# ytinyui/music2midi

Measured on AMD Instinct MI355X. Metric: decoded MIDI tokens/sec/node on 10 s clips, higher is better.
Workload: dtype bf16; 1 GPU; BASELINE configs[2]: full generate (log-mel + encoder + KV-cached greedy decode), bf16, batch 32 clips/GPU x 220500 samples, S=864, max_length 1024; global_batch=32, clips_per_gpu=32, rows_with_eos=0, parallelism=clip-sharded x1, weight_broadcast_bytes=0, world=1, backend=none

## Files before the change

music2midi_amd/csrc/decode.hip:

```cpp
#include "mma.h"
#include "t5.h"

#include <stdlib.h>
#include <type_traits>

namespace m2m {

#ifdef M2M_STAMPS
__device__ unsigned long long g_stamps[1 << 18];
__device__ unsigned int g_stamp_n;
#define M2M_STAMP(kid, phase)                                                                   \
  do {                                                                                          \
    if (threadIdx.x == 0 && blockIdx.x == 0 && blockIdx.y == 0) {                               \
      static_assert((phase) < 8, "phase");                                                      \
      if ((phase) == 0) m2m_stamp_base = atomicAdd(&g_stamp_n, 8u);                             \
      const unsigned long long tk = __builtin_amdgcn_s_memrealtime();                           \
      if (m2m_stamp_base + 8 <= (1u << 18))                                                     \
        g_stamps[m2m_stamp_base + (phase)] = ((unsigned long long)(kid) << 56) | ((unsigned long long)(phase) << 48) | (tk & 0xFFFFFFFFFFFFull); \
    }                                                                                           \
  } while (0)
#define M2M_STAMP_DECL unsigned int m2m_stamp_base = 0; (void)m2m_stamp_base;
#else
#define M2M_STAMP(kid, phase) do {} while (0)
#define M2M_STAMP_DECL
// ... 519 lines not shown
  int H, inner;
  DecState* state;
  const float* emb;
  unsigned long long* keys;
  int* finished;
  int64_t* tokens;
  const int* tok_row;
  int max_len, V, pad_id, eos_id;
  int book;
  const int* fin_skip;
  int fin_stride;
  const unsigned char* anc;
  int64_t anc_par;
  int anc_ld;
  int beam_nb;
};

typedef unsigned int m2m_u32x4 __attribute__((ext_vector_type(4)));
template <bool NT, typename V> __device__ inline V kv_load(const V* p) {
  if constexpr (NT) return __builtin_bit_cast(V, __builtin_nontemporal_load(reinterpret_cast<const m2m_u32x4*>(p)));
  else return *p;
}
#define M2M_KV_LOAD(p) kv_load<NT>(p)

template <typename T> __device__ inline float m2m_exp(float x) {
  if constexpr (sizeof(T) == 2) return __builtin_amdgcn_exp2f(x * 1.4426950408889634f);
  else return expf(x);
}

typedef __bf16 m2m_bf16x2 __attribute__((ext_vector_type(2)));
// ... 80 lines not shown
    if (lane == 0) red.lf[wave] = red.l[wave] * fw;
  }
  __syncthreads();
  if (tid < DK) {
    float s = 0.f, L = 0.f;
#pragma unroll
    for (int wv = 0; wv < 16; ++wv) {
      s += red.o[wv][tid];
      L += red.lf[wv];
    }
    put_in<T>(oh, tid, !(L <= 0.f) ? s / L : 0.f);
  }
  __syncthreads();
}

template <typename T, int C, int LPO, int WREG>
__device__ __forceinline__ void da_project(float (&acc)[C], const Vec16<T> (&w)[WREG], const T* wrow, int cnt, int part, const float* hn, int d) {
  constexpr int E = 16 / sizeof(T);
  using V16 = decltype(Vec16<T>().v);
#pragma unroll
  for (int c = 0; c < C; ++c) acc[c] = 0.f;
#pragma unroll
  for (int u = 0; u < WREG; ++u) {
    if (u < cnt) {
#pragma unroll
      for (int c = 0; c < C; ++c) acc[c] = chunk_dot<T>(w[u], hn + c * d, u * LPO + part, acc[c]);
    }
  }
  for (int i = WREG; i < cnt; i += 4) {
    Vec16<T> w2[4];
// ... 36 lines not shown
}

__device__ __forceinline__ void da_book_row(const DecAttnArgs& a, int b, int st_t, int st_done) {
  if (!st_done) {
    const int fin = a.finished[b];
    const int next = amax_key_token(a.keys[b], fin, a.V, a.pad_id);
    if (st_t < a.max_len) a.tokens[(int64_t)a.tok_row[b] * a.max_len + st_t] = next;
    const int nf = fin | (next == a.eos_id);
    a.finished[b] = nf;
    if (!nf) atomicAdd(&a.state->n_unfinished, 1);
    a.keys[b] = 0ull;
  }
  if (b == 0) a.state->t_copy = st_t;
}

template <typename T, bool SELF, bool NT, bool FETCH = false, bool BEAM = false>
__global__ __launch_bounds__(1024) void dec_attn_kernel(DecAttnArgs a) {
  static_assert(!FETCH || SELF, "only the layer-0 self-attention fetches its input row from the embedding table");
  static_assert(!(FETCH && BEAM), "the beam step is not headless");
  constexpr int E = 16 / sizeof(T);
  constexpr int LPR = DK / E;
  constexpr int KPW = 64 / LPR;
  constexpr int KPB = 16 * KPW;
  constexpr int NOUT = DK;
  constexpr int LPO = 16;
  constexpr int LPO2 = 8;
  constexpr int WMAX2 = 6;
#ifndef M2M_DA_PF_CROSS
#define M2M_DA_PF_CROSS 2
#endif
#ifndef M2M_DA_PF_SELF
#define M2M_DA_PF_SELF 2
#endif
#ifndef M2M_DA_REQUEST_FIRST
// ... 23 lines not shown
  const int hh = blockIdx.x, b = blockIdx.y;
  const int row_fin = a.fin_skip[(int64_t)b * a.fin_stride];
  const int sub = lane % LPR;
  const int kslot = wave * KPW + lane / LPR;
  const int bkv = (BEAM && !SELF) ? b / a.beam_nb : b;
  T* Kb = reinterpret_cast<T*>(a.Kc) + ((int64_t)bkv * a.H + hh) * a.kv_stride * DK;
  T* Vb = reinterpret_cast<T*>(a.Vc) + ((int64_t)bkv * a.H + hh) * a.kv_stride * DK;
  unsigned char* const ancl = reinterpret_cast<unsigned char*>(hn + a.d + (SELF ? a.bias_stride : 0));
  const int beam = (BEAM && SELF) ? b % a.beam_nb : 0;
  if constexpr (BEAM && SELF) {
    const unsigned char* ar = a.anc + (int64_t)(st_t & 1) * a.anc_par + (int64_t)b * a.anc_ld;
    const int na = min(max(st_t, 1), a.kv_stride);
    for (int j = tid; j < na; j += 1024) ancl[j] = j < st_t ? (unsigned char)min((int)ar[j], a.beam_nb - 1) : (unsigned char)beam;
    __syncthreads();
  }
  auto kvoff = [&](int key) -> int64_t {
    int64_t o = (int64_t)key * DK + sub * E;
    if constexpr (BEAM && SELF) o += ((int64_t)ancl[key] - beam) * ((int64_t)a.H * a.kv_stride * DK);
    return o;
  };

  const int xc = min(tid * 4, a.d - 4);
  const int on_ = min(tid >> 1, a.d - 1), opart = tid & 1;
  longlong2 xr0 = make_longlong2(0, 0), xr1 = make_longlong2(0, 0);
  xq_t xres = 0;
  unsigned long long kraw = 0;
  int fin0 = 0;
  if constexpr (FETCH) {
    kraw = a.keys[b];
    fin0 = a.finished[b];
  } else {
    xr0 = *reinterpret_cast<const longlong2*>(a.x + (int64_t)b * a.d + xc);
    xr1 = *reinterpret_cast<const longlong2*>(a.x + (int64_t)b * a.d + xc + 2);
    xres = a.x[(int64_t)b * a.d + on_];
  }
  const float4 gv = *reinterpret_cast<const float4*>(a.ln_w + xc);
  __builtin_amdgcn_sched_barrier(0);
  const int po = min(tid / LPO, NOUT - 1), part = tid % LPO;
  const int which = po / DK, dd = po - which * DK;
  const T* wrow = reinterpret_cast<const T*>(a.Wp) + ((int64_t)which * a.inner + hh * DK + dd) * a.d;
  const int cnt = a.d / E / LPO;
  Vec16<T> w[WMAX];
#pragma unroll
  for (int u = 0; u < WMAX; ++u) w[u].v = *reinterpret_cast<const V16*>(wrow + (min(u, cnt - 1) * LPO + part) * E);
  float* const biasl = hn + a.d;
  constexpr int BPT = 2;
  float bv[SELF ? BPT : 1];
  if (SELF) {
#pragma unroll
    for (int u = 0; u < BPT; ++u) bv[u] = a.bias[(int64_t)hh * a.bias_stride + min(tid + 1024 * u, a.bias_stride - 1)];
  }

  const int t = SELF ? (a.self_len_override > 0 ? a.self_len_override - 1 : st_t) : 0;
  const int n_prev = SELF ? t : a.n_keys;
  const int last = max(n_prev - 1, 0);

  Vec16<T> kv[PF], vv[PF];
#pragma unroll
  for (int u = 0; u < PF; ++u) {
    const int64_t off = kvoff(min(kslot + u * KPB, last));
    kv[u].v = M2M_KV_LOAD(reinterpret_cast<const V16*>(Kb + off));
    vv[u].v = M2M_KV_LOAD(reinterpret_cast<const V16*>(Vb + off));
  }
  __builtin_amdgcn_sched_barrier(0);
  const bool own_wave = wave * 256 < a.d;
  float4 xv = make_float4(0.f, 0.f, 0.f, 0.f);
  float eres = 0.f;
  float4 e4 = make_float4(0.f, 0.f, 0.f, 0.f);
  if constexpr (FETCH) {
    const int tok = amax_key_token(kraw, fin0, a.V, a.pad_id);
    const float* er = a.emb + (int64_t)tok * a.d;
    e4 = *reinterpret_cast<const float4*>(er + xc);
    eres = er[on_];
  }
  {
    const bool own = tid * 4 < a.d;
    if (own_wave) {
      if constexpr (FETCH) xv = e4;
      else xv = make_float4(xq_flt(xr0.x), xq_flt(xr0.y), xq_flt(xr1.x), xq_flt(xr1.y));
      float ss = own ? (xv.x * xv.x + xv.y * xv.y + xv.z * xv.z + xv.w * xv.w) : 0.f;
      ss = wave_sum(ss);
      if (lane == 0) redw[wave] = ss;
    } else if (lane == 0) {
      redw[wave] = 0.f;
    }
    __syncthreads();
    M2M_STAMP(6 + (SELF ? 1 : 0), 4);
    if (own) {
      float tot = 0.f;
#pragma unroll
      for (int wv = 0; wv < 16; ++wv) tot += redw[wv];
      const float rs = rsqrtf(tot / (float)a.d + a.eps);
      put_in<T>(hn, xc + 0, gv.x * (xv.x * rs));
      put_in<T>(hn, xc + 1, gv.y * (xv.y * rs));
      put_in<T>(hn, xc + 2, gv.z * (xv.z * rs));
      put_in<T>(hn, xc + 3, gv.w * (xv.w * rs));
    }
    __syncthreads();
    M2M_STAMP(6 + (SELF ? 1 : 0), 5);
  }

  {
    float q[1];
    da_project<T, 1, LPO>(q, w, wrow, cnt, part, hn, a.d);
#ifndef M2M_STAMPS_MERGE
    M2M_STAMP(6 + (SELF ? 1 : 0), 6);
#endif
    if (part == 0 && tid < NOUT * LPO) qs[dd] = q[0];
  }
  if (SELF) {
#pragma unroll
    for (int u = 0; u < BPT; ++u)
      if (tid + 1024 * u < a.bias_stride) biasl[tid + 1024 * u] = bv[u];
    for (int n = tid + 1024 * BPT; n < a.bias_stride; n += 1024) biasl[n] = a.bias[(int64_t)hh * a.bias_stride + n];
  }
  __syncthreads();
  M2M_STAMP(6 + (SELF ? 1 : 0), 1);

  constexpr int OCH = 32 / E;
  const T* woimg = reinterpret_cast<const T*>(a.Wo) + ((int64_t)hh * OCH * 2 * a.d + min(tid, 2 * a.d - 1)) * E;
  Vec16<T> wo[OCH];
#pragma unroll
  for (int u = 0; u < OCH; ++u) wo[u].v = *reinterpret_cast<const V16*>(woimg + (int64_t)u * 2 * a.d * E);
  const int o2 = tid >> 3, part2 = tid & 7;
  const int which2 = 1 + (o2 >> 6), dd2 = o2 & 63;
  const T* wrow2 = reinterpret_cast<const T*>(a.Wp) + ((int64_t)which2 * a.inner + hh * DK + dd2) * a.d;
  const int cnt2 = a.d / E / LPO2;
  Vec16<T> wkv[SELF ? WMAX2 : 1];
  if (SELF) {
#pragma unroll
    for (int u = 0; u < WMAX2; ++u) wkv[u].v = *reinterpret_cast<const V16*>(wrow2 + (min(u, cnt2 - 1) * LPO2 + part2) * E);
  }

  const int n_live = row_fin ? 0 : n_prev;
  float qv[E];
#pragma unroll
  for (int e = 0; e < E; ++e) qv[e] = qs[sub * E + e];
  DaSoftmax<T> sm;
  auto round = [&](const int k0, const int u, Vec16<T>& ks, Vec16<T>& vs, const int reissue ) {
    const int key = k0 + kslot + u * KPB;
    float s = 0.f;
#pragma unroll
    for (int e = 0; e < E; ++e) s = fmaf(qv[e], ks.get(e), s);
    s = group_sum<LPR>(s);
#if M2M_DA_REQUEST_FIRST
    float vrow[E];
#pragma unroll
    for (int e = 0; e < E; ++e) vrow[e] = vs.get(e);
    if (reissue == 1 || (reissue == 2 && k0 + (u + PF) * KPB < n_live)) {
      const int64_t off = kvoff(min(key + PF * KPB, last));
      ks.v = M2M_KV_LOAD(reinterpret_cast<const V16*>(Kb + off));
      vs.v = M2M_KV_LOAD(reinterpret_cast<const V16*>(Vb + off));
    }
    if (key < n_live) {
      if (SELF) s += biasl[t - key];
      sm.visit(s, vrow);
    }
#else
    if (key < n_live) {
      float vrow[E];
#pragma unroll
      for (int e = 0; e < E; ++e) vrow[e] = vs.get(e);
      if (SELF) s += biasl[t - key];
      sm.visit(s, vrow);
    }
    if (reissue == 1 || (reissue == 2 && k0 + (u + PF) * KPB < n_live)) {
      const int64_t off = kvoff(min(key + PF * KPB, last));
      ks.v = M2M_KV_LOAD(reinterpret_cast<const V16*>(Kb + off));
      vs.v = M2M_KV_LOAD(reinterpret_cast<const V16*>(Vb + off));
    }
#endif
  };
  int k0 = 0;
  for (; k0 + (2 * PF - 1) * KPB < n_live; k0 += PF * KPB) {
#pragma unroll
    for (int u = 0; u < PF; ++u) round(k0, u, kv[u], vv[u], 1);
  }
  for (; k0 < n_live; k0 += PF * KPB) {
#pragma unroll
    for (int u = 0; u < PF; ++u) round(k0, u, kv[u], vv[u], 2);
  }
  if (SELF) {
    float kvn[1];
    da_project<T, 1, LPO2>(kvn, wkv, wrow2, cnt2, part2, hn, a.d);
    if (part2 == 0) da_append_kv<T>(kvn[0], 0, which2, dd2, t, 0, Kb, Vb, kn, vn, !st_done);
    __syncthreads();
  }
  if (SELF && wave == 0 && lane < LPR) sm.visit_own(qv, kn, vn, biasl, sub);
  M2M_STAMP(6 + (SELF ? 1 : 0), 2);

  da_merge<T>(sm, red, oh, [&] {
#ifdef M2M_STAMPS_MERGE
    M2M_STAMP(6 + (SELF ? 1 : 0), 6);
#endif
  });
  M2M_STAMP(6 + (SELF ? 1 : 0), 7);
  da_out_row<T>(a, wo, oh, b, !st_done, true, [&] { return FETCH ? xq_fix_guarded(eres, a.state) : xres; });
  if (!SELF && a.book && hh == 0 && tid == 0) da_book_row(a, b, st_t, st_done);
  M2M_STAMP(6 + (SELF ? 1 : 0), 3);
}

#ifndef M2M_MC_PF_SELF
#define M2M_MC_PF_SELF 2
#endif
#ifndef M2M_MC_PF_CROSS
#define M2M_MC_PF_CROSS 2
#endif
#ifndef M2M_MC_ABL
#define M2M_MC_ABL 0
#endif
#ifndef M2M_MC_WAVES
#define M2M_MC_WAVES 4
#endif
template <typename T, bool SELF, bool NT, bool FETCH, int C, int CIF = 1, bool BEAM = false>
// ... 394 lines not shown
    else launch(s, no, fetch, beam);
  };
  if (a.beam_nb > 0) {
    if (self) by_nt(yes, no, yes);
    else by_nt(no, no, yes);
  } else if (self && a.emb) {
    by_nt(yes, yes, no);
  } else if (self) {
    by_nt(yes, no, no);
  } else {
    by_nt(no, no, no);
  }
}

template <typename T>
static void launch_dec_attn_t(bool self, bool nt, const DecAttnArgs& a, dim3 grid, size_t smem, hipStream_t st) {
  launch_dec_attn_form(self, nt, a, [&](auto s, auto n, auto f, auto bm) {
    hipLaunchKernelGGL((dec_attn_kernel<T, s.value, n.value, f.value, bm.value>), grid, dim3(1024), smem, st, a);
  });
}

template <typename T, int C>
static void launch_dec_attn_mc_t(bool self, bool nt, const DecAttnArgs& a, int nb, int cif, size_t smem, hipStream_t st) {
  const dim3 grid((unsigned)a.H, (unsigned)ceil_div(nb, C));
  launch_dec_attn_form(self, nt, a, [&](auto s, auto n, auto f, auto bm) {
    if constexpr (!s.value && !bm.value) {
      if (cif == 2) {
        hipLaunchKernelGGL((dec_attn_mc_kernel<T, false, n.value, false, C, 2>), grid, dim3(1024), smem, st, a, nb);
        return;
      }
    }
    hipLaunchKernelGGL((dec_attn_mc_kernel<T, s.value, n.value, f.value, C, 1, bm.value>), grid, dim3(1024), smem, st, a, nb);
  });
}

static int launch_dec_attn(int precision, bool self, bool nt, DecAttnArgs a, int B, int clips, int cif, hipStream_t st) {
  size_t smem = ((size_t)a.d * (size_t)clips + (self ? (size_t)a.bias_stride : 0)) * sizeof(float);
  if (self && a.beam_nb > 0) smem += (size_t)clips * a.kv_stride;
  M2M_REQUIRE(smem <= 24 * 1024, "decode attention: max_dec_len=%d too long for the LDS bias row%s (<= %d)", a.bias_stride,
              self && a.beam_nb > 0 ? " and ancestries" : "",
              (24 * 1024 - a.d * 4 * clips) / (self && a.beam_nb > 0 ? 4 + clips : 4));
  const bool bf = precision == M2M_PREC_BF16;
  if (clips == 1) {
    dim3 grid((unsigned)a.H, (unsigned)B);
    if (bf) launch_dec_attn_t<bf16_t>(self, nt, a, grid, smem, st);
    else launch_dec_attn_t<float>(self, nt, a, grid, smem, st);
  } else if (clips == 2) {
    if (bf) launch_dec_attn_mc_t<bf16_t, 2>(self, nt, a, B, cif, smem, st);
    else launch_dec_attn_mc_t<float, 2>(self, nt, a, B, cif, smem, st);
  } else if (clips == 4) {
    if (bf) launch_dec_attn_mc_t<bf16_t, 4>(self, nt, a, B, cif, smem, st);
    else launch_dec_attn_mc_t<float, 4>(self, nt, a, B, cif, smem, st);
  } else {
    set_error("decode attention: %d clips per workgroup not instantiated (1, 2, 4)", clips);
    return M2M_ERR_INVALID;
  }
  M2M_CHECK_HIP(hipGetLastError());
  return M2M_OK;
}

struct DecHeadArgs {
// ... 1023 lines not shown
    a.beam_nb = s->beam_nb;
    a.anc = s->anc + (int64_t)v.b0 * s->max_dec; a.anc_par = (int64_t)s->max_batch * s->max_dec; a.anc_ld = s->max_dec;
  }
  if (headless && layer == 0) {
    a.keys = s->keys + v.b0; a.finished = s->finished + v.b0; a.tokens = s->tokens; a.tok_row = s->tok_row + v.b0;
    a.max_len = s->max_dec; a.V = g.vocab_size; a.pad_id = g.pad_token_id; a.eos_id = g.eos_token_id;
    if (self) a.emb = m->shared; else a.book = 1;
  }
  if (self) {
    const size_t off = ((size_t)layer * kv_layer_elems(s, s->max_dec) + (size_t)v.b0 * H * s->max_dec * DK) * es;
    a.ln_w = L.ln0; a.Wp = L.wqkv; a.Wo = L.wo_img;
    a.Kc = (unsigned char*)s->self_k + off;
    a.Vc = (unsigned char*)s->self_v + off;
    a.kv_stride = s->max_dec; a.n_keys = 0; a.self_len_override = self_len;
    a.bias = s->dec_bias_tab; a.bias_stride = s->max_dec;
    return launch_dec_attn(m->precision, true, nt, a, v.nb, clips, s->sw.mc_cif, st);
  }
  const size_t per = (size_t)s->B * H * s->S * DK;
  const size_t voff = (size_t)(beam ? v.b0 / s->beam_nb : v.b0) * H * s->S * DK;
  a.ln_w = L.ln1; a.Wp = L.wcq; a.Wo = L.wco_img;
  a.Kc = (unsigned char*)s->cross_kv + (((size_t)layer * 2 + 0) * per + voff) * es;
  a.Vc = (unsigned char*)s->cross_kv + (((size_t)layer * 2 + 1) * per + voff) * es;
  a.kv_stride = s->S; a.n_keys = s->S; a.self_len_override = 0; a.bias = nullptr; a.bias_stride = 0;
  return launch_dec_attn(m->precision, false, nt, a, v.nb, clips, s->sw.mc_cif, st);
}

int decode_launch_step(m2m_session* s, const DecView& v, bool forced, float* logits_out, int Ld, hipStream_t st) {
  const m2m_model* m = s->m;
  const m2m_t5_geometry& g = m->g;
  const int P = m->precision;
  xq_t* xA = xbuf(s, v, 0);
  xq_t* xB = xbuf(s, v, 1);
  xq_t* xC = xbuf(s, v, 2);
  int rc;
  const bool headless = headless_for(s, forced);
  for (int l = 0; l < g.num_decoder_layers; ++l) {
    const DecLayerPacked& L = m->dec[l];
    if ((rc = decode_launch_attn(s, v, true, l, 0, st, headless, !forced))) return rc;
    if ((rc = decode_launch_attn(s, v, false, l, 0, st, headless, !forced))) return rc;
// ... 41 lines not shown
```

music2midi_amd/csrc/t5.h:

```cpp
#pragma once

#include "common.h"
#include "env.h"

#include <vector>

namespace m2m {

constexpr int DK = 64;

struct EncLayerPacked {
  const float* ln0;
  const void* wqkv;
  const void* wo;
  const float* ln1;
  const void* wi;
  const void* wo_ff;
};

struct DecLayerPacked {
  const float* ln0;
  const void* wqkv;
  const void* wo;
  const float* ln1;
  const void* wcq;
  const void* wco;
  const float* ln2;
  const void* wi;
  const void* wo_ff;
  const void* ff_img;
  const void* wo_img;
  const void* wco_img;
};

constexpr int FF_IMG_FRAG = 512;
constexpr int FF_IMG_WAVE = 12 * FF_IMG_FRAG;

}

struct m2m_model {
  m2m_t5_geometry g;
  int precision;
  int inner;
  int vocab_pad;
  size_t esize;
  void* blob = nullptr;
  int64_t blob_bytes = 0;
  std::vector<m2m::EncLayerPacked> enc;
  std::vector<m2m::DecLayerPacked> dec;
  const float* enc_final_ln = nullptr;
  const float* dec_final_ln = nullptr;
  const float* shared = nullptr;
  const void* lm_head = nullptr;
  const void* wckv = nullptr;
  std::vector<float> enc_rel_bias_host;
  std::vector<float> dec_rel_bias_host;
};

namespace m2m {

struct DecState {
  int t;
  int done;
  int out_len;
  int n_unfinished;
  int max_steps;
  int overflow;
  int t_copy;
  int zero;
// ... 117 lines not shown
inline const EncSwitches& enc_switches_now() { return tl_enc_switches ? *tl_enc_switches : process_enc_switches(); }

struct SessionSwitches {
  static int one_of_124(int c) { return (c == 1 || c == 2 || c == 4) ? c : 0; }
  static int zero_is_1(int c) { return c == 0 ? 1 : c; }
  EncSwitches enc = read_enc_switches();
  int attn_clips = env_int("M2M_DA_CLIPS", 0);
  int attn_clips_self = one_of_124(env_int("M2M_DA_CLIPS_SELF", 0));
  int ff_rows = env_int("M2M_DEC_FF_ROWS", 0);
  int ff_slices = env_int("M2M_DEC_FF_SLICES", 0);
  int mc_cif = zero_is_1(env_int("M2M_MC_CIF", 0));
  bool headless = env_on("M2M_HEADLESS");
  bool finished_skip = env_on("M2M_FINISHED_SKIP");
  int kv_resident_layers = env_int("M2M_KV_RESIDENT_LAYERS", -1);
  bool kv_resident_stagger = env_on("M2M_KV_RESIDENT_STAGGER");
};

constexpr int MAX_GROUPS = 8;

struct DecView {
  int b0, nb;
  DecState* state;
  int ord = 0, count = 1;
};

inline bool kv_layer_resident(int layer, int L, int resident, int ord, int count, bool stagger) {
  if (resident >= L) return true;
  if (resident <= 0) return false;
  const int first = (stagger && count == 2) ? (ord * resident) % L : 0;
  return (layer - first + L) % L < resident;
}

struct DecGroup {
  DecView view{0, 0, nullptr};
  DecState* state_host = nullptr;
  hipStream_t stream = nullptr;
  hipEvent_t ev_done = nullptr;
  hipGraphExec_t graph_exec = nullptr;
  struct GraphEntry { int key[10]; hipGraph_t graph; hipGraphExec_t exec; unsigned long long used; };
  std::vector<GraphEntry> graphs;
  unsigned long long graph_clock = 0;
};
}

struct m2m_session {
  const m2m_model* m;
  int max_batch, max_enc, max_dec;
  unsigned char* ws;
  int64_t ws_bytes;
  float* x_enc;
  void* h_enc;
  void* qkv_enc;
  void* vt_enc;
  void* attn_enc;
// ... 81 lines not shown
};
int launch_attn(int precision, const AttnArgs& a, bool causal, hipStream_t st);
int launch_transpose_v(int precision, const void* v, void* vt, int BH, int S, int Sp, hipStream_t st);
int launch_embed_rows(const int64_t* ids, const float* table, float* x, int M, int d, int V, int pad_id, hipStream_t st);
int launch_final_norm_f32(const float* x, const float* w, float* out_f32, void* out_T, int precision, int M, int d,
                          float eps, hipStream_t st);

int launch_convert(int precision, const float* src, void* dst, int64_t n, hipStream_t st);
int launch_interleave(int precision, const float* wi0, const float* wi1, void* dst, int dff, int d, int half,
                      hipStream_t st);
int launch_ff_image(int precision, const void* wi, const void* wo_ff, void* img, int dff, int d, hipStream_t st);
int launch_attn_out_image(int precision, const void* wo, void* img, int H, int d, hipStream_t st);
int launch_copy_f32(const float* src, float* dst, int64_t n, hipStream_t st);
int launch_fill_zero(void* dst, int64_t bytes, hipStream_t st);
int launch_checksum(const void* buf, int64_t bytes, unsigned long long* acc_dev, hipStream_t st);

int decode_init(m2m_session* s, const DecView& v, int max_steps, bool forced, hipStream_t st);
int decode_launch_step(m2m_session* s, const DecView& v, bool forced, float* logits_out, int Ld, hipStream_t st);
int decode_launch_attn(m2m_session* s, const DecView& v, bool self, int layer, int self_len, hipStream_t st, bool headless = false,
                       bool skip_finished = false);
int decode_move_rows(m2m_session* s, const int* src, const int* dst, int n, int t, hipStream_t st);
struct KvPolicy { bool nt; int resident; };
KvPolicy decode_kv_policy(const m2m_session* s);
bool decode_chains_may_drift(const m2m_session* s, int chains);
int decode_clear_self(m2m_session* s, const DecView& v, int t0, int t1, hipStream_t st);
int decode_finalize(m2m_session* s, const DecView& v, hipStream_t st);
constexpr int HEAD_GREEDY = 0, HEAD_SAMPLE = 1, HEAD_BEAM = 2;
constexpr int HEAD_PROCESSED = 4;
constexpr int HEAD_SCORED = 8;
constexpr int BEAM_MAX = 32;
// ... 9 lines not shown
```

music2midi_amd/csrc/t5_api.hip:

```cpp
#include "carver.h"
#include "env.h"
#include "t5.h"

#include <math.h>
#include <stdlib.h>
#include <string.h>
#include <algorithm>
#include <memory>
#include <vector>

using namespace m2m;

extern "C" int m2m_rel_bucket(int rel, int bidirectional, int num_buckets, int max_distance) {
  int bucket = 0;
  int nb = num_buckets;
  int n;
  if (bidirectional) {
    nb /= 2;
    if (rel > 0) bucket += nb;
    n = rel < 0 ? -rel : rel;
  } else {
    n = rel < 0 ? -rel : 0;
  }
  const int max_exact = nb / 2;
// ... 40 lines not shown
  auto T = [&](const void*& member, int64_t elems) { c.take(member, elems * es); };
  for (EncLayerPacked& L : m->enc) {
    F(L.ln0, d); T(L.wqkv, (int64_t)3 * inner * d); T(L.wo, (int64_t)d * inner);
    F(L.ln1, d); T(L.wi, (int64_t)2 * dff * d); T(L.wo_ff, (int64_t)d * dff);
  }
  for (DecLayerPacked& L : m->dec) {
    F(L.ln0, d); T(L.wqkv, (int64_t)3 * inner * d); T(L.wo, (int64_t)d * inner);
    F(L.ln1, d); T(L.wcq, (int64_t)inner * d); T(L.wco, (int64_t)d * inner);
    F(L.ln2, d); T(L.wi, (int64_t)2 * dff * d); T(L.wo_ff, (int64_t)d * dff); T(L.ff_img, (int64_t)3 * dff * d);
    T(L.wo_img, (int64_t)d * inner); T(L.wco_img, (int64_t)d * inner);
  }
  F(m->enc_final_ln, d); F(m->dec_final_ln, d);
  F(m->shared, (int64_t)V * d);
  T(m->lm_head, (int64_t)vocab_pad * d);
  T(m->wckv, (int64_t)Ld * 2 * inner * d);
  m->blob_bytes = c.off;
  hipError_t e = hipMalloc(&m->blob, (size_t)c.off);
  if (e != hipSuccess) {
    set_error("m2m_model_create: hipMalloc(%lld) failed: %s", (long long)c.off, hipGetErrorString(e));
    delete m;
    return M2M_ERR_NOMEM;
  }
  c.bind((unsigned char*)m->blob);
  int rc = M2M_OK;
  if (hipMemsetAsync(m->blob, 0, (size_t)c.off, st) != hipSuccess) { set_error("m2m_model_create: hipMemsetAsync failed"); rc = M2M_ERR_HIP; }
  auto at = [&](const void* member, int64_t part = 0) { return (unsigned char*)const_cast<void*>(member) + part * inner * d * (int64_t)es; };
  auto conv = [&](const float* src, void* dst, int64_t n) {
    if (rc == M2M_OK && !src) { set_error("m2m_model_create: null layer weight pointer"); rc = M2M_ERR_INVALID; }
    if (rc == M2M_OK) rc = launch_convert(precision, src, dst, n, st);
  };
// ... 21 lines not shown
    conv(s.q, at(L.wqkv, 0), (int64_t)inner * d); conv(s.k, at(L.wqkv, 1), (int64_t)inner * d); conv(s.v, at(L.wqkv, 2), (int64_t)inner * d);
    conv(s.o, at(L.wo), (int64_t)d * inner);
    conv(s.cq, at(L.wcq), (int64_t)inner * d);
    conv(s.co, at(L.wco), (int64_t)d * inner);
    if (rc == M2M_OK) rc = launch_attn_out_image(precision, L.wo, at(L.wo_img), g.num_heads, d, st);
    if (rc == M2M_OK) rc = launch_attn_out_image(precision, L.wco, at(L.wco_img), g.num_heads, d, st);
    interleave(s.wi0, s.wi1, L.wi, 8);
    conv(s.wo, at(L.wo_ff), (int64_t)d * dff);
    if (rc == M2M_OK) rc = launch_ff_image(precision, L.wi, L.wo_ff, at(L.ff_img), dff, d, st);
    conv(s.ck, at(m->wckv, l * 2 + 0), (int64_t)inner * d); conv(s.cv, at(m->wckv, l * 2 + 1), (int64_t)inner * d);
  }
  copyf(w->enc_final_ln, m->enc_final_ln, d); copyf(w->dec_final_ln, m->dec_final_ln, d);
  copyf(w->shared, m->shared, (int64_t)V * d);
  if (rc == M2M_OK) rc = launch_fill_zero(at(m->lm_head), (int64_t)vocab_pad * d * es, st);
  conv(w->lm_head, at(m->lm_head), (int64_t)V * d);
  m->enc_rel_bias_host.resize((size_t)g.num_buckets * g.num_heads);
  m->dec_rel_bias_host.resize((size_t)g.num_buckets * g.num_heads);
  hipError_t he = hipSuccess;
  if (rc == M2M_OK) he = hipMemcpyAsync(m->enc_rel_bias_host.data(), w->enc_rel_bias, m->enc_rel_bias_host.size() * 4, hipMemcpyDeviceToHost, st);
  if (rc == M2M_OK && he == hipSuccess) he = hipMemcpyAsync(m->dec_rel_bias_host.data(), w->dec_rel_bias, m->dec_rel_bias_host.size() * 4, hipMemcpyDeviceToHost, st);
  if (rc == M2M_OK && he == hipSuccess) he = hipStreamSynchronize(st);
  if (rc == M2M_OK && he != hipSuccess) { set_error("m2m_model_create: %s", hipGetErrorString(he)); rc = M2M_ERR_HIP; }
  if (rc != M2M_OK) {
    (void)hipFree(m->blob);
    delete m;
    return rc;
  }
  *out = m;
  return M2M_OK;
}
// ... 61 lines not shown
  c.take(s->hyp_tok, (int64_t)B * L * 8);
  c.take(s->score_dev, sizeof(ScoreParams));
  c.take(s->gram_dev, sizeof(GrammarParams));
  c.take(s->gram_state, (int64_t)B * sizeof(GrammarState));
}

int check_switches(const SessionSwitches& sw) {
  M2M_REQUIRE(sw.attn_clips == 0 || sw.attn_clips == 1 || sw.attn_clips == 2 || sw.attn_clips == 4,
              "M2M_DA_CLIPS=%d: clips per decode-attention workgroup must be 0 (by chain size), 1, 2 or 4", sw.attn_clips);
  M2M_REQUIRE(sw.ff_rows == 0 || sw.ff_rows == 8 || sw.ff_rows == 16,
              "M2M_DEC_FF_ROWS=%d: rows per decode feed-forward workgroup must be 0 (by chain size), 8 or 16", sw.ff_rows);
  M2M_REQUIRE(sw.ff_slices == 0 || sw.ff_slices == 1 || sw.ff_slices == 2 || sw.ff_slices == 4,
              "M2M_DEC_FF_SLICES=%d: hidden slices per decode feed-forward workgroup must be 0 (by chain size), 1, 2 or 4", sw.ff_slices);
  M2M_REQUIRE(sw.mc_cif == 1 || sw.mc_cif == 2,
              "M2M_MC_CIF=%d: clips in flight in the multi-clip cross-attention must be 0 (default: 1), 1 or 2", sw.mc_cif);
  return M2M_OK;
}

hipError_t upload_bias_tables(m2m_session* s) {
  const m2m_model* m = s->m;
  const m2m_t5_geometry& g = m->g;
  const int H = g.num_heads, S = s->max_enc, L = s->max_dec;
  std::vector<float> et((size_t)H * (2 * S - 1)), dt((size_t)H * L);
  for (int rel = -(S - 1); rel <= S - 1; ++rel) {
    const int bk = m2m_rel_bucket(rel, 1, g.num_buckets, g.max_distance);
    for (int h = 0; h < H; ++h) et[(size_t)h * (2 * S - 1) + rel + S - 1] = m->enc_rel_bias_host[(size_t)bk * H + h];
  }
  for (int n = 0; n < L; ++n) {
    const int bk = m2m_rel_bucket(-n, 0, g.num_buckets, g.max_distance);
    for (int h = 0; h < H; ++h) dt[(size_t)h * L + n] = m->dec_rel_bias_host[(size_t)bk * H + h];
// ... 207 lines not shown
  if (G > MAX_GROUPS) G = MAX_GROUPS;
  const int unit = s->beam_nb > 0 ? s->beam_nb : 1, units = nrows / unit;
  if (G > units) G = units;
  const int base = units / G, extra = units % G;
  int b0 = 0;
  for (int i = 0; i < G; ++i) {
    s->groups[i].view.b0 = b0;
    s->groups[i].view.nb = (base + (i < extra ? 1 : 0)) * unit;
    s->groups[i].view.ord = i; s->groups[i].view.count = G;
    b0 += s->groups[i].view.nb;
  }
  return G;
}

static int ensure_graph(m2m_session* s, DecGroup& gr, int steps) {
  const int key[10] = {s->B, s->S, gr.view.b0, gr.view.nb, steps, s->sw.finished_skip ? 1 : 0, s->head_mode, s->beam_nb,
                       gr.view.ord, gr.view.count};
  ++gr.graph_clock;
  for (auto& ge : gr.graphs)
    if (memcmp(key, ge.key, sizeof(key)) == 0) { ge.used = gr.graph_clock; gr.graph_exec = ge.exec; return M2M_OK; }
  constexpr size_t MAX_CACHED = 12;
  if (gr.graphs.size() >= MAX_CACHED) {
    size_t lru = 0;
    for (size_t i = 1; i < gr.graphs.size(); ++i) if (gr.graphs[i].used < gr.graphs[lru].used) lru = i;
    (void)hipGraphExecDestroy(gr.graphs[lru].exec);
    (void)hipGraphDestroy(gr.graphs[lru].graph);
    gr.graphs.erase(gr.graphs.begin() + (long)lru);
  }
  gr.graph_exec = nullptr;
  M2M_CHECK_HIP(hipStreamBeginCapture(gr.stream, hipStreamCaptureModeThreadLocal));
  int rc = M2M_OK;
  for (int i = 0; i < steps && rc == M2M_OK; ++i) rc = decode_launch_step(s, gr.view, false, nullptr, 0, gr.stream);
// ... 611 lines not shown
```

Baseline: 178,200 tokens/s.

## Precompute per-token layer-0 q/k/v tables and gather cached K/V by token

At the first decoder layer the input row is just the token embedding, so RMS norm and the q/k/v projections depend only on the token id. A load-time kernel precomputes per-head q, k, v tables over the vocabulary. The layer-0 self-attention then looks up this step's q/k/v instead of projecting, and in form 2 gathers past keys and values from the tables via the row's token history rather than the KV cache. This removes the weight loads and matvecs from the layer-0 step, at the cost of extra model memory, a token-history read into LDS, and scattered table gathers.

```diff
diff --git a/music2midi_amd/csrc/decode.hip b/music2midi_amd/csrc/decode.hip
--- a/music2midi_amd/csrc/decode.hip
+++ b/music2midi_amd/csrc/decode.hip
@@ -557,6 +557,9 @@
   int64_t anc_par;
   int anc_ld;
   int beam_nb;
+  const float* q0_tab;
+  const void* k0_tab;
+  const void* v0_tab;
 };
 
 typedef unsigned int m2m_u32x4 __attribute__((ext_vector_type(4)));
@@ -667,6 +670,35 @@
   __syncthreads();
 }
 
+template <typename T, typename Row, typename Mid>
+__device__ __forceinline__ void da_norm_row(Row row, const float4& gv, int xc, int d, float eps, float* redw, float* hn, Mid mid) {
+  const int tid = threadIdx.x, lane = tid & 63, wave = tid >> 6;
+  const bool own_wave = wave * 256 < d;
+  const bool own = tid * 4 < d;
+  float4 xv = make_float4(0.f, 0.f, 0.f, 0.f);
+  if (own_wave) {
+    xv = row();
+    float ss = own ? (xv.x * xv.x + xv.y * xv.y + xv.z * xv.z + xv.w * xv.w) : 0.f;
+    ss = wave_sum(ss);
+    if (lane == 0) redw[wave] = ss;
+  } else if (lane == 0) {
+    redw[wave] = 0.f;
+  }
+  __syncthreads();
+  mid();
+  if (own) {
+    float tot = 0.f;
+#pragma unroll
+    for (int wv = 0; wv < 16; ++wv) tot += redw[wv];
+    const float rs = rsqrtf(tot / (float)d + eps);
+    put_in<T>(hn, xc + 0, gv.x * (xv.x * rs));
+    put_in<T>(hn, xc + 1, gv.y * (xv.y * rs));
+    put_in<T>(hn, xc + 2, gv.z * (xv.z * rs));
+    put_in<T>(hn, xc + 3, gv.w * (xv.w * rs));
+  }
+  __syncthreads();
+}
+
 template <typename T, int C, int LPO, int WREG>
 __device__ __forceinline__ void da_project(float (&acc)[C], const Vec16<T> (&w)[WREG], const T* wrow, int cnt, int part, const float* hn, int d) {
   constexpr int E = 16 / sizeof(T);
@@ -733,10 +765,13 @@
   if (b == 0) a.state->t_copy = st_t;
 }
 
-template <typename T, bool SELF, bool NT, bool FETCH = false, bool BEAM = false>
+template <typename T, bool SELF, bool NT, bool FETCH = false, bool BEAM = false, int TAB = 0>
 __global__ __launch_bounds__(1024) void dec_attn_kernel(DecAttnArgs a) {
   static_assert(!FETCH || SELF, "only the layer-0 self-attention fetches its input row from the embedding table");
   static_assert(!(FETCH && BEAM), "the beam step is not headless");
+  static_assert(TAB == 0 || FETCH, "the token tables serve the headless layer-0 self-attention: its input row is emb[tok] itself");
+  constexpr bool TABLE = TAB > 0;
+  constexpr bool NTS = NT && TAB != 2;
   constexpr int E = 16 / sizeof(T);
   constexpr int LPR = DK / E;
   constexpr int KPW = 64 / LPR;
@@ -790,11 +825,15 @@
     for (int j = tid; j < na; j += 1024) ancl[j] = j < st_t ? (unsigned char)min((int)ar[j], a.beam_nb - 1) : (unsigned char)beam;
     __syncthreads();
   }
+  unsigned short* const tokl = reinterpret_cast<unsigned short*>(hn + a.d + (SELF ? a.bias_stride : 0));
   auto kvoff = [&](int key) -> int64_t {
+    if constexpr (TAB == 2) return (int64_t)tokl[key] * DK + sub * E;
     int64_t o = (int64_t)key * DK + sub * E;
     if constexpr (BEAM && SELF) o += ((int64_t)ancl[key] - beam) * ((int64_t)a.H * a.kv_stride * DK);
     return o;
   };
+  const T* const Ks = TAB == 2 ? reinterpret_cast<const T*>(a.k0_tab) + (int64_t)hh * a.V * DK : Kb;
+  const T* const Vs = TAB == 2 ? reinterpret_cast<const T*>(a.v0_tab) + (int64_t)hh * a.V * DK : Vb;
 
   const int xc = min(tid * 4, a.d - 4);
   const int on_ = min(tid >> 1, a.d - 1), opart = tid & 1;
@@ -802,23 +841,34 @@
   xq_t xres = 0;
   unsigned long long kraw = 0;
   int fin0 = 0;
+  const int64_t* hrow = nullptr;
   if constexpr (FETCH) {
     kraw = a.keys[b];
     fin0 = a.finished[b];
+    if constexpr (TABLE) hrow = a.tokens + (int64_t)a.tok_row[b] * a.max_len;
   } else {
     xr0 = *reinterpret_cast<const longlong2*>(a.x + (int64_t)b * a.d + xc);
     xr1 = *reinterpret_cast<const longlong2*>(a.x + (int64_t)b * a.d + xc + 2);
     xres = a.x[(int64_t)b * a.d + on_];
   }
-  const float4 gv = *reinterpret_cast<const float4*>(a.ln_w + xc);
+  constexpr int HPT = 2;
+  int64_t hv[TAB == 2 ? HPT : 1];
+  if constexpr (TAB == 2) {
+#pragma unroll
+    for (int u = 0; u < HPT; ++u) hv[u] = hrow[min(tid + 1024 * u, max(st_t - 1, 0))];
+  }
+  float4 gv = make_float4(0.f, 0.f, 0.f, 0.f);
+  if constexpr (!TABLE) gv = *reinterpret_cast<const float4*>(a.ln_w + xc);
   __builtin_amdgcn_sched_barrier(0);
   const int po = min(tid / LPO, NOUT - 1), part = tid % LPO;
   const int which = po / DK, dd = po - which * DK;
   const T* wrow = reinterpret_cast<const T*>(a.Wp) + ((int64_t)which * a.inner + hh * DK + dd) * a.d;
   const int cnt = a.d / E / LPO;
-  Vec16<T> w[WMAX];
-#pragma unroll
-  for (int u = 0; u < WMAX; ++u) w[u].v = *reinterpret_cast<const V16*>(wrow + (min(u, cnt - 1) * LPO + part) * E);
+  Vec16<T> w[TABLE ? 1 : WMAX];
+  if constexpr (!TABLE) {
+#pragma unroll
+    for (int u = 0; u < WMAX; ++u) w[u].v = *reinterpret_cast<const V16*>(wrow + (min(u, cnt - 1) * LPO + part) * E);
+  }
   float* const biasl = hn + a.d;
   constexpr int BPT = 2;
   float bv[SELF ? BPT : 1];
@@ -832,24 +882,42 @@
   const int last = max(n_prev - 1, 0);
 
   Vec16<T> kv[PF], vv[PF];
-#pragma unroll
-  for (int u = 0; u < PF; ++u) {
-    const int64_t off = kvoff(min(kslot + u * KPB, last));
-    kv[u].v = M2M_KV_LOAD(reinterpret_cast<const V16*>(Kb + off));
-    vv[u].v = M2M_KV_LOAD(reinterpret_cast<const V16*>(Vb + off));
+  if constexpr (TAB != 2) {
+#pragma unroll
+    for (int u = 0; u < PF; ++u) {
+      const int64_t off = kvoff(min(kslot + u * KPB, last));
+      kv[u].v = kv_load<NTS>(reinterpret_cast<const V16*>(Ks + off));
+      vv[u].v = kv_load<NTS>(reinterpret_cast<const V16*>(Vs + off));
+    }
   }
   __builtin_amdgcn_sched_barrier(0);
   const bool own_wave = wave * 256 < a.d;
   float4 xv = make_float4(0.f, 0.f, 0.f, 0.f);
   float eres = 0.f;
   float4 e4 = make_float4(0.f, 0.f, 0.f, 0.f);
+  int tok = 0;
   if constexpr (FETCH) {
-    const int tok = amax_key_token(kraw, fin0, a.V, a.pad_id);
+    tok = amax_key_token(kraw, fin0, a.V, a.pad_id);
     const float* er = a.emb + (int64_t)tok * a.d;
-    e4 = *reinterpret_cast<const float4*>(er + xc);
+    if constexpr (!TABLE) e4 = *reinterpret_cast<const float4*>(er + xc);
     eres = er[on_];
   }
-  {
+  if constexpr (TABLE) {
+    const int64_t trow = ((int64_t)hh * a.V + tok) * DK;
+    const int dd2 = tid & 63, which2 = 1 + ((tid >> 6) & 1);
+    const float qe = a.q0_tab[trow + dd2];
+    const T kve = (which2 == 1 ? reinterpret_cast<const T*>(a.k0_tab) : reinterpret_cast<const T*>(a.v0_tab))[trow + dd2];
+    if (tid < DK) qs[dd2] = qe;
+    if (tid < 2 * DK) da_append_kv<T>(to_f32(kve), 0, which2, dd2, t, 0, Kb, Vb, kn, vn, !st_done);
+    if constexpr (TAB == 2) {
+      const int nh = max(t, 1);
+#pragma unroll
+      for (int u = 0; u < HPT; ++u)
+        if (tid + 1024 * u < nh) tokl[tid + 1024 * u] = (unsigned short)min(max(hv[u], (int64_t)0), (int64_t)a.V - 1);
+      for (int n = tid + 1024 * HPT; n < nh; n += 1024) tokl[n] = (unsigned short)min(max(hrow[min(n, last)], (int64_t)0), (int64_t)a.V - 1);
+    }
+  }
+  if constexpr (!TABLE) {
     const bool own = tid * 4 < a.d;
     if (own_wave) {
       if constexpr (FETCH) xv = e4;
@@ -876,7 +944,7 @@
     M2M_STAMP(6 + (SELF ? 1 : 0), 5);
   }
 
-  {
+  if constexpr (!TABLE) {
     float q[1];
     da_project<T, 1, LPO>(q, w, wrow, cnt, part, hn, a.d);
 #ifndef M2M_STAMPS_MERGE
@@ -892,6 +960,14 @@
   }
   __syncthreads();
   M2M_STAMP(6 + (SELF ? 1 : 0), 1);
+  if constexpr (TAB == 2) {
+#pragma unroll
+    for (int u = 0; u < PF; ++u) {
+      const int64_t off = kvoff(min(kslot + u * KPB, last));
+      kv[u].v = kv_load<NTS>(reinterpret_cast<const V16*>(Ks + off));
+      vv[u].v = kv_load<NTS>(reinterpret_cast<const V16*>(Vs + off));
+    }
+  }
 
   constexpr int OCH = 32 / E;
   const T* woimg = reinterpret_cast<const T*>(a.Wo) + ((int64_t)hh * OCH * 2 * a.d + min(tid, 2 * a.d - 1)) * E;
@@ -902,8 +978,8 @@
   const int which2 = 1 + (o2 >> 6), dd2 = o2 & 63;
   const T* wrow2 = reinterpret_cast<const T*>(a.Wp) + ((int64_t)which2 * a.inner + hh * DK + dd2) * a.d;
   const int cnt2 = a.d / E / LPO2;
-  Vec16<T> wkv[SELF ? WMAX2 : 1];
-  if (SELF) {
+  Vec16<T> wkv[SELF && !TABLE ? WMAX2 : 1];
+  if (SELF && !TABLE) {
 #pragma unroll
     for (int u = 0; u < WMAX2; ++u) wkv[u].v = *reinterpret_cast<const V16*>(wrow2 + (min(u, cnt2 - 1) * LPO2 + part2) * E);
   }
@@ -925,8 +1001,8 @@
     for (int e = 0; e < E; ++e) vrow[e] = vs.get(e);
     if (reissue == 1 || (reissue == 2 && k0 + (u + PF) * KPB < n_live)) {
       const int64_t off = kvoff(min(key + PF * KPB, last));
-      ks.v = M2M_KV_LOAD(reinterpret_cast<const V16*>(Kb + off));
-      vs.v = M2M_KV_LOAD(reinterpret_cast<const V16*>(Vb + off));
+      ks.v = kv_load<NTS>(reinterpret_cast<const V16*>(Ks + off));
+      vs.v = kv_load<NTS>(reinterpret_cast<const V16*>(Vs + off));
     }
     if (key < n_live) {
       if (SELF) s += biasl[t - key];
@@ -942,8 +1018,8 @@
     }
     if (reissue == 1 || (reissue == 2 && k0 + (u + PF) * KPB < n_live)) {
       const int64_t off = kvoff(min(key + PF * KPB, last));
-      ks.v = M2M_KV_LOAD(reinterpret_cast<const V16*>(Kb + off));
-      vs.v = M2M_KV_LOAD(reinterpret_cast<const V16*>(Vb + off));
+      ks.v = kv_load<NTS>(reinterpret_cast<const V16*>(Ks + off));
+      vs.v = kv_load<NTS>(reinterpret_cast<const V16*>(Vs + off));
     }
 #endif
   };
@@ -956,7 +1032,7 @@
 #pragma unroll
     for (int u = 0; u < PF; ++u) round(k0, u, kv[u], vv[u], 2);
   }
-  if (SELF) {
+  if constexpr (SELF && !TABLE) {
     float kvn[1];
     da_project<T, 1, LPO2>(kvn, wkv, wrow2, cnt2, part2, hn, a.d);
     if (part2 == 0) da_append_kv<T>(kvn[0], 0, which2, dd2, t, 0, Kb, Vb, kn, vn, !st_done);
@@ -974,6 +1050,58 @@
   da_out_row<T>(a, wo, oh, b, !st_done, true, [&] { return FETCH ? xq_fix_guarded(eres, a.state) : xres; });
   if (!SELF && a.book && hh == 0 && tid == 0) da_book_row(a, b, st_t, st_done);
   M2M_STAMP(6 + (SELF ? 1 : 0), 3);
+}
+
+template <typename T>
+__global__ __launch_bounds__(1024) void dec_token_tables_kernel(const float* __restrict__ emb, const float* __restrict__ ln_w, const T* __restrict__ Wp,
+                                                                int d, int inner, int V, float eps, float* __restrict__ q0, T* __restrict__ k0,
+                                                                T* __restrict__ v0) {
+  constexpr int E = 16 / sizeof(T), NOUT = DK, LPO = 16, LPO2 = 8, WMAX = 3, WMAX2 = 6;
+  using V16 = decltype(Vec16<T>().v);
+  extern __shared__ __align__(16) float hn[];
+  __shared__ float redw[16];
+  const int tid = threadIdx.x, hh = blockIdx.x, tok = blockIdx.y;
+  const int xc = min(tid * 4, d - 4);
+  const float4 gv = *reinterpret_cast<const float4*>(ln_w + xc);
+  const float4 e4 = *reinterpret_cast<const float4*>(emb + (int64_t)tok * d + xc);
+  const int po = min(tid / LPO, NOUT - 1), part = tid % LPO;
+  const int which = po / DK, dd = po - which * DK;
+  const T* wrow = Wp + ((int64_t)which * inner + hh * DK + dd) * d;
+  const int cnt = d / E / LPO;
+  Vec16<T> w[WMAX];
+#pragma unroll
+  for (int u = 0; u < WMAX; ++u) w[u].v = *reinterpret_cast<const V16*>(wrow + (min(u, cnt - 1) * LPO + part) * E);
+  const int o2 = tid >> 3, part2 = tid & 7;
+  const int which2 = 1 + (o2 >> 6), dd2 = o2 & 63;
+  const T* wrow2 = Wp + ((int64_t)which2 * inner + hh * DK + dd2) * d;
+  const int cnt2 = d / E / LPO2;
+  Vec16<T> wkv[WMAX2];
+#pragma unroll
+  for (int u = 0; u < WMAX2; ++u) wkv[u].v = *reinterpret_cast<const V16*>(wrow2 + (min(u, cnt2 - 1) * LPO2 + part2) * E);
+  da_norm_row<T>([&] { return e4; }, gv, xc, d, eps, redw, hn, [] {});
+  const int64_t trow = ((int64_t)hh * V + tok) * DK;
+  float q[1], kvn[1];
+  da_project<T, 1, LPO>(q, w, wrow, cnt, part, hn, d);
+  if (part == 0 && tid < NOUT * LPO) q0[trow + dd] = q[0];
+  da_project<T, 1, LPO2>(kvn, wkv, wrow2, cnt2, part2, hn, d);
+  if (part2 == 0) (which2 == 1 ? k0 : v0)[trow + dd2] = from_f32<T>(kvn[0]);
+}
+
+int launch_token_tables(const m2m_model* m, hipStream_t st) {
+  if (!m->q0_tab) return M2M_OK;
+  const m2m_t5_geometry& g = m->g;
+  const DecLayerPacked& L = m->dec[0];
+  const dim3 grid((unsigned)g.num_heads, (unsigned)g.vocab_size);
+  const size_t smem = (size_t)g.d_model * sizeof(float);
+  float* q0 = const_cast<float*>(m->q0_tab);
+  if (m->precision == M2M_PREC_BF16)
+    hipLaunchKernelGGL(dec_token_tables_kernel<bf16_t>, grid, dim3(1024), smem, st, m->shared, L.ln0, (const bf16_t*)L.wqkv, g.d_model, m->inner,
+                       g.vocab_size, g.layer_norm_eps, q0, (bf16_t*)const_cast<void*>(m->k0_tab), (bf16_t*)const_cast<void*>(m->v0_tab));
+  else
+    hipLaunchKernelGGL(dec_token_tables_kernel<float>, grid, dim3(1024), smem, st, m->shared, L.ln0, (const float*)L.wqkv, g.d_model, m->inner,
+                       g.vocab_size, g.layer_norm_eps, q0, (float*)const_cast<void*>(m->k0_tab), (float*)const_cast<void*>(m->v0_tab));
+  M2M_CHECK_HIP(hipGetLastError());
+  return M2M_OK;
 }
 
 #ifndef M2M_MC_PF_SELF
@@ -1398,8 +1526,12 @@
 }
 
 template <typename T>
-static void launch_dec_attn_t(bool self, bool nt, const DecAttnArgs& a, dim3 grid, size_t smem, hipStream_t st) {
+static void launch_dec_attn_t(bool self, bool nt, int tab, const DecAttnArgs& a, dim3 grid, size_t smem, hipStream_t st) {
   launch_dec_attn_form(self, nt, a, [&](auto s, auto n, auto f, auto bm) {
+    if constexpr (f.value) {
+      if (tab == 1) { hipLaunchKernelGGL((dec_attn_kernel<T, true, n.value, true, false, 1>), grid, dim3(1024), smem, st, a); return; }
+      if (tab == 2) { hipLaunchKernelGGL((dec_attn_kernel<T, true, n.value, true, false, 2>), grid, dim3(1024), smem, st, a); return; }
+    }
     hipLaunchKernelGGL((dec_attn_kernel<T, s.value, n.value, f.value, bm.value>), grid, dim3(1024), smem, st, a);
   });
 }
@@ -1418,17 +1550,20 @@
   });
 }
 
-static int launch_dec_attn(int precision, bool self, bool nt, DecAttnArgs a, int B, int clips, int cif, hipStream_t st) {
+static int launch_dec_attn(int precision, bool self, bool nt, int tab, DecAttnArgs a, int B, int clips, int cif, hipStream_t st) {
   size_t smem = ((size_t)a.d * (size_t)clips + (self ? (size_t)a.bias_stride : 0)) * sizeof(float);
   if (self && a.beam_nb > 0) smem += (size_t)clips * a.kv_stride;
+  M2M_REQUIRE(tab == 0 || (self && clips == 1 && a.beam_nb == 0 && a.emb && a.q0_tab && a.k0_tab && a.v0_tab && a.tokens && a.tok_row),
+              "decode attention: the token-table form %d needs the one-clip headless layer-0 self-attention, the model's tables and the row's tokens", tab);
+  if (tab == 2) smem += ((size_t)a.kv_stride * 2 + 3) / 4 * 4;
   M2M_REQUIRE(smem <= 24 * 1024, "decode attention: max_dec_len=%d too long for the LDS bias row%s (<= %d)", a.bias_stride,
               self && a.beam_nb > 0 ? " and ancestries" : "",
               (24 * 1024 - a.d * 4 * clips) / (self && a.beam_nb > 0 ? 4 + clips : 4));
   const bool bf = precision == M2M_PREC_BF16;
   if (clips == 1) {
     dim3 grid((unsigned)a.H, (unsigned)B);
-    if (bf) launch_dec_attn_t<bf16_t>(self, nt, a, grid, smem, st);
-    else launch_dec_attn_t<float>(self, nt, a, grid, smem, st);
+    if (bf) launch_dec_attn_t<bf16_t>(self, nt, tab, a, grid, smem, st);
+    else launch_dec_attn_t<float>(self, nt, tab, a, grid, smem, st);
   } else if (clips == 2) {
     if (bf) launch_dec_attn_mc_t<bf16_t, 2>(self, nt, a, B, cif, smem, st);
     else launch_dec_attn_mc_t<float, 2>(self, nt, a, B, cif, smem, st);
@@ -2482,7 +2617,10 @@
     a.Vc = (unsigned char*)s->self_v + off;
     a.kv_stride = s->max_dec; a.n_keys = 0; a.self_len_override = self_len;
     a.bias = s->dec_bias_tab; a.bias_stride = s->max_dec;
-    return launch_dec_attn(m->precision, true, nt, a, v.nb, clips, s->sw.mc_cif, st);
+    int tab = 0;
+    if (layer == 0 && clips == 1 && !beam && self_len <= 0 && m->q0_tab && a.emb) tab = s->sw.token_tables;
+    if (tab) { a.q0_tab = m->q0_tab; a.k0_tab = m->k0_tab; a.v0_tab = m->v0_tab; }
+    return launch_dec_attn(m->precision, true, nt, tab, a, v.nb, clips, s->sw.mc_cif, st);
   }
   const size_t per = (size_t)s->B * H * s->S * DK;
   const size_t voff = (size_t)(beam ? v.b0 / s->beam_nb : v.b0) * H * s->S * DK;
@@ -2490,7 +2628,7 @@
   a.Kc = (unsigned char*)s->cross_kv + (((size_t)layer * 2 + 0) * per + voff) * es;
   a.Vc = (unsigned char*)s->cross_kv + (((size_t)layer * 2 + 1) * per + voff) * es;
   a.kv_stride = s->S; a.n_keys = s->S; a.self_len_override = 0; a.bias = nullptr; a.bias_stride = 0;
-  return launch_dec_attn(m->precision, false, nt, a, v.nb, clips, s->sw.mc_cif, st);
+  return launch_dec_attn(m->precision, false, nt, 0, a, v.nb, clips, s->sw.mc_cif, st);
 }
 
 int decode_launch_step(m2m_session* s, const DecView& v, bool forced, float* logits_out, int Ld, hipStream_t st) {
diff --git a/music2midi_amd/csrc/t5.h b/music2midi_amd/csrc/t5.h
--- a/music2midi_amd/csrc/t5.h
+++ b/music2midi_amd/csrc/t5.h
@@ -35,6 +35,7 @@
 
 constexpr int FF_IMG_FRAG = 512;
 constexpr int FF_IMG_WAVE = 12 * FF_IMG_FRAG;
+constexpr int64_t TOKEN_TABLES_MAX_BYTES = 16ll << 20;
 
 }
 
@@ -53,6 +54,9 @@
   const float* shared = nullptr;
   const void* lm_head = nullptr;
   const void* wckv = nullptr;
+  const float* q0_tab = nullptr;
+  const void* k0_tab = nullptr;
+  const void* v0_tab = nullptr;
   std::vector<float> enc_rel_bias_host;
   std::vector<float> dec_rel_bias_host;
 };
@@ -200,6 +204,7 @@
   bool finished_skip = env_on("M2M_FINISHED_SKIP");
   int kv_resident_layers = env_int("M2M_KV_RESIDENT_LAYERS", -1);
   bool kv_resident_stagger = env_on("M2M_KV_RESIDENT_STAGGER");
+  int token_tables = env_int("M2M_DEC_TOKEN_TABLES", 2);
 };
 
 constexpr int MAX_GROUPS = 8;
@@ -223,7 +228,7 @@
   hipStream_t stream = nullptr;
   hipEvent_t ev_done = nullptr;
   hipGraphExec_t graph_exec = nullptr;
-  struct GraphEntry { int key[10]; hipGraph_t graph; hipGraphExec_t exec; unsigned long long used; };
+  struct GraphEntry { int key[11]; hipGraph_t graph; hipGraphExec_t exec; unsigned long long used; };
   std::vector<GraphEntry> graphs;
   unsigned long long graph_clock = 0;
 };
@@ -335,6 +340,7 @@
 int launch_copy_f32(const float* src, float* dst, int64_t n, hipStream_t st);
 int launch_fill_zero(void* dst, int64_t bytes, hipStream_t st);
 int launch_checksum(const void* buf, int64_t bytes, unsigned long long* acc_dev, hipStream_t st);
+int launch_token_tables(const m2m_model* m, hipStream_t st);
 
 int decode_init(m2m_session* s, const DecView& v, int max_steps, bool forced, hipStream_t st);
 int decode_launch_step(m2m_session* s, const DecView& v, bool forced, float* logits_out, int Ld, hipStream_t st);
diff --git a/music2midi_amd/csrc/t5_api.hip b/music2midi_amd/csrc/t5_api.hip
--- a/music2midi_amd/csrc/t5_api.hip
+++ b/music2midi_amd/csrc/t5_api.hip
@@ -78,6 +78,9 @@
   F(m->shared, (int64_t)V * d);
   T(m->lm_head, (int64_t)vocab_pad * d);
   T(m->wckv, (int64_t)Ld * 2 * inner * d);
+  const int64_t tab_elems = (int64_t)g.num_heads * V * DK;
+  const bool tables = V <= 65535 && tab_elems * (int64_t)(4 + 2 * es) <= TOKEN_TABLES_MAX_BYTES;
+  if (tables) { F(m->q0_tab, tab_elems); T(m->k0_tab, tab_elems); T(m->v0_tab, tab_elems); }
   m->blob_bytes = c.off;
   hipError_t e = hipMalloc(&m->blob, (size_t)c.off);
   if (e != hipSuccess) {
@@ -129,6 +132,7 @@
   copyf(w->shared, m->shared, (int64_t)V * d);
   if (rc == M2M_OK) rc = launch_fill_zero(at(m->lm_head), (int64_t)vocab_pad * d * es, st);
   conv(w->lm_head, at(m->lm_head), (int64_t)V * d);
+  if (rc == M2M_OK && tables) rc = launch_token_tables(m, st);
   m->enc_rel_bias_host.resize((size_t)g.num_buckets * g.num_heads);
   m->dec_rel_bias_host.resize((size_t)g.num_buckets * g.num_heads);
   hipError_t he = hipSuccess;
@@ -220,6 +224,8 @@
               "M2M_DEC_FF_SLICES=%d: hidden slices per decode feed-forward workgroup must be 0 (by chain size), 1, 2 or 4", sw.ff_slices);
   M2M_REQUIRE(sw.mc_cif == 1 || sw.mc_cif == 2,
               "M2M_MC_CIF=%d: clips in flight in the multi-clip cross-attention must be 0 (default: 1), 1 or 2", sw.mc_cif);
+  M2M_REQUIRE(sw.token_tables >= 0 && sw.token_tables <= 2,
+              "M2M_DEC_TOKEN_TABLES=%d: the layer-0 token-table form must be 0 (off), 1 (this step's q, k, v) or 2 (and the cached K/V)", sw.token_tables);
   return M2M_OK;
 }
 
@@ -457,8 +463,9 @@
 }
 
 static int ensure_graph(m2m_session* s, DecGroup& gr, int steps) {
-  const int key[10] = {s->B, s->S, gr.view.b0, gr.view.nb, steps, s->sw.finished_skip ? 1 : 0, s->head_mode, s->beam_nb,
-                       gr.view.ord, gr.view.count};
+  const int key[11] = {s->B, s->S, gr.view.b0, gr.view.nb, steps, s->sw.finished_skip ? 1 : 0, s->head_mode, s->beam_nb,
+                       gr.view.ord, gr.view.count,
+                       s->sw.token_tables};
   ++gr.graph_clock;
   for (auto& ge : gr.graphs)
     if (memcmp(key, ge.key, sizeof(key)) == 0) { ge.used = gr.graph_clock; gr.graph_exec = ge.exec; return M2M_OK; }
```

Result: faster. 182,300 tokens/s (median of 6 runs) (+2.3%).
